# RIVM-bioinformatics/TrueConsense

Measured on NVIDIA B200. Metric: aligned_bases_per_sec_pileup_consensus, higher is better.
Workload: dtype int32

## Files before the change

### trueconsense_b200/csrc/cuda/call.cu

```cuda
#include <stdlib.h>

#include "tc_common.cuh"

__device__ __forceinline__ double pct(int c, int cov) { return __dmul_rn(__ddiv_rn((double)c, (double)cov), 100.0); }
__device__ __forceinline__ bool within(double a, double b, double maxdist) { return fabs(__dsub_rn(a, b)) <= maxdist; }

struct ranked5 { int cnt[5]; char let[5]; };

__device__ __forceinline__ void rank5(const int c[5], ranked5& r) {
    const int asc[5] = {'A', 'T', 'C', 'G', 'X'};
#pragma unroll
    for (int i = 0; i < 5; ++i) {
        int beat = 0;
#pragma unroll
        for (int j = 0; j < 5; ++j)
            if (j != i && (c[j] > c[i] || (c[j] == c[i] && asc[j] > asc[i]))) ++beat;
#pragma unroll
        for (int k = 0; k < 5; ++k)
            if (beat == k) { r.cnt[k] = c[i]; r.let[k] = (char)asc[i]; }
    }
}

__device__ __forceinline__ char iupac_of_mask(int m) {
    switch (m) {
// ... 126 lines not shown
    nn = min(nn, end);
    xrun[j] = nn - k;
    if (nn == end) flags[j] |= TC_CF_XRUN_OFF_END;
}

__global__ void is_ambiguous_kernel(const uint8_t* __restrict__ letters, const int32_t* __restrict__ cnts,
                                    const int32_t* __restrict__ cov, int64_t n, double maxdist, uint8_t* __restrict__ out) {
    int64_t i = (int64_t)blockIdx.x * blockDim.x + threadIdx.x;
    if (i >= n) return;
    char let[4]; int cnt[4];
#pragma unroll
    for (int k = 0; k < 4; ++k) { let[k] = (char)letters[k * n + i]; cnt[k] = cnts[k * n + i]; }
    out[i] = (uint8_t)is_ambiguous(let, cnt, cov[i], maxdist);
}

__global__ void list_candidates_kernel(const uint8_t* __restrict__ flags, int L, int32_t* __restrict__ out, int cap, int32_t* __restrict__ n_out) {
    const int j = blockIdx.x * blockDim.x + threadIdx.x;
    if (j < L && (flags[j] & TC_CF_INS_CANDIDATE)) {
        const int slot = atomicAdd(n_out, 1);
        if (slot < cap) out[slot] = j + 1;
    }
}

__global__ void rank_sort_kernel(const int32_t* __restrict__ in, const int32_t* __restrict__ n_in, int cap, int32_t* __restrict__ out) {
    const int n = min(*n_in, cap);
    for (int i = blockIdx.x * blockDim.x + threadIdx.x; i < n; i += gridDim.x * blockDim.x) {
        const int v = in[i];
        int rank = 0;
        for (int k = 0; k < n; ++k) rank += in[k] < v;
        out[rank] = v;
    }
}

static int call_table(tc_ctx_t* ctx, const int32_t* counts, int32_t ref_len, const int32_t* d_contig_start, int32_t n_contigs,
                      const tc_call_params_t* p, const tc_call_table_t* t, cudaStream_t s) {
    const size_t L = (size_t)ref_len;
    int rc;
    call_args a;
    a.counts = (const int32_t*)tc_stage_in(ctx, SLOT_COUNTS, counts, sizeof(int32_t) * TC_NROWS * L, s, &rc);
    if (rc) return rc;
    a.L = ref_len; a.mincov = p->mincov; a.include_ambig = p->include_ambig;
    a.maxdist = p->ambig_maxdist; a.mdel_pct = p->minority_del_pct; a.ins_pct = p->insert_pct;
    struct out_t { void* user; void* dev; size_t bytes; int slot; };
    out_t outs[6] = {
        {t->call_char, nullptr, L, SLOT_CALL_A}, {t->flags, nullptr, L, SLOT_CALL_B}, {t->xrun, nullptr, 4 * L, SLOT_CALL_C},
        {t->rank_letter, nullptr, 4 * L, SLOT_CALL_D}, {t->rank_count, nullptr, 16 * L, SLOT_CALL_E}, {t->ambig_char, nullptr, L, SLOT_CALL_F}};
// ... 79 lines not shown
    const int32_t* dc = (const int32_t*)tc_stage_in(ctx, SLOT_TMP_B, cnts, 16 * (size_t)n, s, &rc); if (rc) return rc;
    const int32_t* dv = (const int32_t*)tc_stage_in(ctx, SLOT_TMP_C, cov, 4 * (size_t)n, s, &rc); if (rc) return rc;
    bool out_dev = tc_is_device_ptr(out_char);
    uint8_t* d_out = out_dev ? out_char : (uint8_t*)tc_dev_buf(ctx, SLOT_CALL_F, (size_t)n);
    if (!d_out) return TC_ERR_NOMEM;
    is_ambiguous_kernel<<<(unsigned)((n + 255) / 256), 256, 0, s>>>(dl, dc, dv, n, maxdist, d_out);
    TC_LAUNCH_CHECK();
    if (!out_dev) {
        TC_D2H(out_char, d_out, (size_t)n, s);
        TC_CUDA(cudaStreamSynchronize(s));
    }
    return TC_OK;
}

int tc_candidates_enqueue(tc_ctx* ctx, const uint8_t* d_flags, int32_t ref_len, int32_t cap, int32_t** d_count, int32_t** d_sorted, cudaStream_t s) {
    int32_t* d_buf = (int32_t*)tc_dev_buf(ctx, SLOT_TMP_B, 4 * (2 * (size_t)cap + 1) + 64);
    if (!d_buf) return TC_ERR_NOMEM;
    int32_t* d_cnt = d_buf + cap;
    TC_CUDA(cudaMemsetAsync(d_cnt, 0, 4, s));
    list_candidates_kernel<<<(unsigned)((ref_len + 255) / 256), 256, 0, s>>>(d_flags, ref_len, d_buf, cap, d_cnt);
    TC_LAUNCH_CHECK();
    rank_sort_kernel<<<32, 256, 0, s>>>(d_buf, d_cnt, cap, d_cnt + 1);
    TC_LAUNCH_CHECK();
    *d_count = d_cnt; *d_sorted = d_cnt + 1;
    return TC_OK;
}

TC_API int tc_list_insert_candidates(tc_ctx_t* ctx, const uint8_t* flags, int32_t ref_len, int32_t* cand_pos, int32_t cap,
                                     int32_t* n_out, void* stream) {
    if (!ctx) return TC_ERR_ARG;
    if (!flags || !cand_pos || !n_out || ref_len <= 0 || cap < 0) return tc_fail(ctx, TC_ERR_ARG, "bad argument");
    cudaStream_t s = (cudaStream_t)stream;
    TC_CUDA(cudaSetDevice(ctx->device));
    int rc;
    const uint8_t* df = (const uint8_t*)tc_stage_in(ctx, SLOT_TMP_A, flags, (size_t)ref_len, s, &rc); if (rc) return rc;
    int32_t *d_cnt, *d_sorted;
    rc = tc_candidates_enqueue(ctx, df, ref_len, cap, &d_cnt, &d_sorted, s);
// ... 21 lines not shown
```

### trueconsense_b200/csrc/cuda/inserts.cu

```cuda
#include <cub/device/device_segmented_radix_sort.cuh>

#include <memory>
#include <new>

#include "tc_common.cuh"

constexpr int INS_TILE = 256;
constexpr uint64_t KEY_NONE = ~0ull;
constexpr int INS_TBL = 4096;
constexpr int INS_BASES_FIXED = 64;

struct ins_args {
    dreads r;
    const int32_t* cand;
    int n_cand;
    const int32_t* n_cand_dev;
    uint32_t flag_filter; int min_mapq, min_bq, ignore_orphans; long long max_depth;
    int32_t span_hint;
    int32_t* range;
    uint32_t* range_off;
    const int64_t* seg_off;
    const int32_t* tile_cand;
    const int32_t* tile_first;
    int32_t* tile_sel;
    int32_t* tile_last;
    uint64_t* ent_key; int32_t* ent_indel; int32_t* ent_qpos; uint8_t* ent_head;
    uint8_t* ent_sel;
    uint8_t* ent_q;
    uint8_t* pair_q; unsigned long long pair_cap; unsigned long long* pair_bump;
    int olap_mode;
    int32_t* seg_count;
    int32_t* pair_any;
    int32_t* overflow;
    const int32_t* layout;
    uint8_t* bases_fixed;
    tc_status* status;
};

__device__ __forceinline__ int ins_ncand(const ins_args& a) { return a.n_cand_dev ? min(*a.n_cand_dev, a.n_cand) : a.n_cand; }

__global__ void max_span_kernel(dreads r, tc_status* status) {
    int64_t i = (int64_t)blockIdx.x * blockDim.x + threadIdx.x;
    int span = 0;
    if (i < r.n) {
        if (i > 0 && r.pos[i] < r.pos[i - 1]) atomicCAS(&status->err, 0, TC_ERR_UNSORTED);
        for (uint32_t k = r.cigar_off[i]; k < r.cigar_off[i + 1]; ++k) {
            uint32_t c = r.cigar[k];
            if (op_consumes_ref(c & 15u)) span += (int)(c >> 4);
        }
    }
    span = __reduce_max_sync(0xffffffffu, span);
    if ((threadIdx.x & 31) == 0 && span > 0) atomicMax(&status->max_span, span);
}

__device__ __forceinline__ int warp_lower_bound(const int32_t* __restrict__ pos, int64_t n, int v, int lane) {
    int64_t lo = 0, hi = n;
    while (hi > lo) {
        const int64_t step = (hi - lo + 31) / 32;
        const int64_t i = lo + (int64_t)lane * step;
        const bool ge = i >= hi || pos[i] >= v;
        const unsigned m = __ballot_sync(0xffffffffu, ge);
        if (m == 0u) { lo = lo + 31 * step + 1; continue; }
        const int first = __ffs(m) - 1;
        if (first == 0) return (int)lo;
        hi = min(hi, lo + (int64_t)first * step);
        lo = lo + (int64_t)(first - 1) * step + 1;
    }
    return (int)lo;
}

__global__ void cand_range_kernel(ins_args a) {
    const int ci = blockIdx.x * (blockDim.x >> 5) + (threadIdx.x >> 5);
    const int lane = threadIdx.x & 31;
    if (ci >= ins_ncand(a)) return;
    const int c = a.cand[ci] - 1;
    const int ms = max(a.span_hint > 0 ? a.span_hint : a.status->max_span, 1);
    const int lo = warp_lower_bound(a.r.pos, a.r.n, c - ms + 1, lane);
    const int hi = max(lo, warp_lower_bound(a.r.pos, a.r.n, c + 1, lane));
    if (lane == 0) {
        a.range[2 * ci] = lo;
        a.range[2 * ci + 1] = hi;
        a.range_off[4 * ci] = a.r.seq_off[lo]; a.range_off[4 * ci + 1] = a.r.seq_off[hi];
        a.range_off[4 * ci + 2] = a.r.cigar_off[lo]; a.range_off[4 * ci + 3] = a.r.cigar_off[hi];
    }
}

__device__ __forceinline__ uint64_t mix_key(uint64_t h, uint64_t v) {
    h ^= v + 0x9e3779b97f4a7c15ull + (h << 6) + (h >> 2);
    h *= 0xff51afd7ed558ccdull;
    h ^= h >> 33;
    return h;
}

__device__ __forceinline__ char base_char_upper(uint32_t code, bool rev) {
// ... 168 lines not shown
#pragma unroll
    for (int o = 1; o < 32; o <<= 1) { const int t = __shfl_up_sync(0xffffffffu, m, o); if (lane >= o) m = max(m, t); }
    int prev = __shfl_up_sync(0xffffffffu, m, 1);
    if (lane == 0) prev = -1;
    if (lane == 31) wlast[warp] = m;
    if (lane == 0) wsum[warp] = __popc(bal);
    __syncthreads();
    long long rank = base_s + __popc(bal & ((1u << lane) - 1));
    prev = max(prev, prev_s);
    for (int w = 0; w < warp; ++w) { rank += wsum[w]; prev = max(prev, wlast[w]); }
    bool admitted = false;
    if (sel) {
        const bool first_at_start = prev < 0 || a.r.pos[prev] != a.r.pos[r];
        admitted = first_at_start || rank < a.max_depth;
    }
    if (a.min_bq > 0) {
        if (r < hi && admitted) a.ent_sel[slot] = (uint8_t)(es | 4);
        return;
    }
    if (emit && !admitted) a.ent_key[slot] = KEY_NONE;
    const int n_adm = __syncthreads_count(emit && admitted);
    if (threadIdx.x == 0 && n_adm) atomicAdd(&a.seg_count[ci], n_adm);
}

__device__ __forceinline__ uint32_t wang_hash(uint32_t key) {
    key += ~(key << 15); key ^= (key >> 10); key += (key << 3); key ^= (key >> 6); key += ~(key << 11); key ^= (key >> 16);
    return key;
}

struct cwalk { const uint32_t* cig; const uint32_t* end; long long icig, iseq, iref; };

__device__ int iref2iseq_set(cwalk& w, long long pos) {
    if (pos < 0) return -1;
    w.icig = 0; w.iseq = 0; w.iref = 0;
    while (w.cig < w.end) {
        const uint32_t cig = *w.cig & 15u; const long long ncig = (long long)(*w.cig >> 4);
// ... 99 lines not shown
        for (uint32_t k = a.r.cigar_off[r]; k < a.r.cigar_off[r + 1]; ++k) { const uint32_t c = a.r.cigar[k]; if (op_consumes_ref(c & 15u)) end += (int)(c >> 4); }
        if (mp >= end) return false;
    }
    return true;
}

__global__ void __launch_bounds__(1024) ins_pair_kernel(ins_args a) {
    extern __shared__ __align__(16) unsigned char pair_smem[];
    unsigned int* tmin = reinterpret_cast<unsigned int*>(pair_smem);
    unsigned int* tmax = tmin + PAIR_TBL;
    unsigned short* tcnt = reinterpret_cast<unsigned short*>(tmax + PAIR_TBL);
    __shared__ int over_s, nadm_s;
    const int ci = blockIdx.x;
    if (ci >= ins_ncand(a)) return;
    if (a.layout && a.layout[2]) return;
    const int64_t off = a.seg_off[ci];
    const int lo = a.range[2 * ci];
    const int n = a.range[2 * ci + 1] - lo;
    const bool pairing = a.olap_mode != 1 && a.r.qname_hash && a.r.mpos && a.r.isize && a.pair_any[ci];
    if (threadIdx.x == 0) { over_s = 0; nadm_s = 0; }
    if (pairing) {
        for (int i = threadIdx.x; i < PAIR_TBL; i += blockDim.x) { tmin[i] = 0u; tmax[i] = 0u; tcnt[i] = 0; }
        __syncthreads();
        auto is_event = [&](int i, bool& push) -> bool {
            const uint8_t es = a.ent_sel[off + i];
            if (!(es & 1)) return false;
            if (!(es & 4)) { push = false; return true; }
            push = true;
            return true;
        };
        for (int pass = 0; pass < 2; ++pass) {
            for (int i = threadIdx.x; i < n; i += blockDim.x) {
                bool push;
                if (!is_event(i, push) || push != (pass == 0)) continue;
                const uint32_t r = (uint32_t)(lo + i);
                if (push && !(a.r.flag[r] & 2u)) continue;
                const unsigned long long k = a.r.qname_hash[r];
                unsigned h = (unsigned)(k ^ (k >> 31)) & (PAIR_TBL - 1);
                int probes = 0;
                for (;;) {
                    const unsigned cur = push ? atomicCAS(&tmin[h], 0u, (unsigned)i + 1u) : tmin[h];
                    if (cur == 0u && !push) break;
                    if (cur == 0u || a.r.qname_hash[lo + cur - 1] == k) {
                        atomicMin(&tmin[h], (unsigned)i + 1u); atomicMax(&tmax[h], (unsigned)i + 1u);
                        atomicAdd(reinterpret_cast<unsigned int*>(tcnt) + (h >> 1), (h & 1) ? 0x10000u : 1u);
                        break;
                    }
                    h = (h + 1) & (PAIR_TBL - 1);
                    if (++probes >= PAIR_TBL * 3 / 4) { over_s = 1; break; }
                }
            }
            __syncthreads();
        }
        __syncthreads();
        if (over_s) { if (threadIdx.x == 0) atomicCAS(&a.status->err, 0, TC_ERR_CAPACITY); return; }
        for (int h = threadIdx.x; h < PAIR_TBL; h += blockDim.x) {
            const int cnt = tcnt[h];
            if (cnt < 2) continue;
            const int first = (int)tmin[h] - 1, last = (int)tmax[h] - 1;
            const unsigned long long k = a.r.qname_hash[lo + first];
            int stored = -1;
            int seen = 0;
            for (int i = first; i <= last && seen < cnt; i = (cnt == 2 && i == first) ? last : i + 1) {
                bool push;
                if (!is_event(i, push)) continue;
                const uint32_t r = (uint32_t)(lo + i);
                if (a.r.qname_hash[r] != k || (push && !(a.r.flag[r] & 2u))) continue;
                ++seen;
                if (!push) { stored = -1; continue; }
                if (!olap_eligible(a, r)) continue;
                bool has_span = false;
                for (uint32_t q = a.r.cigar_off[r]; q < a.r.cigar_off[r + 1] && !has_span; ++q) { const uint32_t c = a.r.cigar[q]; has_span = op_consumes_ref(c & 15u) && (c >> 4) > 0; }
                if (!has_span) continue;
                if (stored < 0) {
                    const int mp = a.r.mpos[r];
                    if (mp >= a.r.pos[r] || ((a.r.flag[r] & 1u) && mp == -1)) stored = i;
                    continue;
                }
                const int64_t sa = off + stored, sb = off + i;
                const uint32_t ra = (uint32_t)(lo + stored);
                const int la = a.r.l_seq[ra], lb = a.r.l_seq[r];
                const unsigned long long at = atomicAdd(a.pair_bump, (unsigned long long)(la + lb));
                if (at + (unsigned long long)(la + lb) <= a.pair_cap) {
                    uint8_t* aq = a.pair_q + at; uint8_t* bq = aq + la;
                    const uint8_t* ga = a.r.qual + 8ull * a.r.seq_off[ra]; const uint8_t* gb = a.r.qual + 8ull * a.r.seq_off[r];
                    for (int q = 0; q < la; ++q) aq[q] = ga[q];
                    for (int q = 0; q < lb; ++q) bq[q] = gb[q];
                    tweak_pair(a, ra, r, aq, bq, a.olap_mode);
                    if ((a.ent_sel[sa] & 2) && a.ent_qpos[sa] < la) a.ent_q[sa] = aq[a.ent_qpos[sa]];
                    if ((a.ent_sel[sb] & 2) && a.ent_qpos[sb] < lb) a.ent_q[sb] = bq[a.ent_qpos[sb]];
                } else atomicOr(a.overflow, 2);
                stored = -1;
            }
        }
        __syncthreads();
    }
    int mine = 0;
    for (int i = threadIdx.x; i < n; i += blockDim.x) {
        const uint8_t es = a.ent_sel[off + i];
        const bool ok = (es & 6) == 6 && (int)a.ent_q[off + i] >= a.min_bq;
        if (!ok) a.ent_key[off + i] = KEY_NONE;
        mine += ok ? 1 : 0;
    }
    mine = __reduce_add_sync(0xffffffffu, mine);
    if ((threadIdx.x & 31) == 0 && mine) atomicAdd(&nadm_s, mine);
    __syncthreads();
    if (threadIdx.x == 0) a.seg_count[ci] = nadm_s;
}

__device__ __forceinline__ bool same_entry(const ins_args& a, int lo, int64_t off, uint32_t e1, uint32_t e2) {
    if (a.ent_head[e1] != a.ent_head[e2] || a.ent_indel[e1] != a.ent_indel[e2]) return false;
// ... 21 lines not shown
        const uint32_t e = (uint32_t)off + (uint32_t)(0xffffffffull - (best & 0xffffffffull));
        out.mode_count = (int32_t)(best >> 32);
        out.first_read = (int32_t)(a.range[2 * ci] + (int64_t)e - off);
        out.head = a.ent_head[e];
        out.indel = a.ent_indel[e];
        out.bases_off = (int64_t)e;
        if (out.indel > 0 && out.indel <= INS_BASES_FIXED) {
            const read_syms rs = read_syms_of(a, (uint32_t)out.first_read);
            const int q = a.ent_qpos[e];
            for (int j = 1; j <= out.indel; ++j) a.bases_fixed[(size_t)ci * INS_BASES_FIXED + j - 1] = sym_char(rs.sym(q + j));
        }
    }
    calls[ci] = out;
}

__global__ void __launch_bounds__(1024) ins_count_kernel(ins_args a, tc_insert_call_t* __restrict__ calls) {
    extern __shared__ __align__(16) unsigned char ins_smem[];
    unsigned long long* tkey = reinterpret_cast<unsigned long long*>(ins_smem);
    unsigned int* tcnt = reinterpret_cast<unsigned int*>(tkey + INS_TBL);
    unsigned int* tfirst = tcnt + INS_TBL;
    __shared__ unsigned long long best_s;
    __shared__ int over_s, hashed_s;
    const int ci = blockIdx.x;
    if (ci >= ins_ncand(a)) return;
    if (a.layout && a.layout[2]) return;
    const int64_t off = a.seg_off[ci];
    const int lo = a.range[2 * ci];
    const int n = a.range[2 * ci + 1] - lo;
    for (int i = threadIdx.x; i < INS_TBL; i += blockDim.x) { tkey[i] = KEY_NONE; tcnt[i] = 0; tfirst[i] = 0xffffffffu; }
    if (threadIdx.x == 0) { best_s = 0ull; over_s = 0; hashed_s = 0; }
    __syncthreads();
    for (int base = 0; base < n; base += 4 * (int)blockDim.x) {
        unsigned long long kk[4];
#pragma unroll
        for (int u = 0; u < 4; ++u) {
            const int i = base + u * (int)blockDim.x + (int)threadIdx.x;
            kk[u] = i < n ? a.ent_key[off + i] : KEY_NONE;
        }
#pragma unroll
        for (int u = 0; u < 4; ++u) {
            const int i = base + u * (int)blockDim.x + (int)threadIdx.x;
            const unsigned long long k = kk[u];
            const unsigned grp = __match_any_sync(0xffffffffu, k);
            if (k == KEY_NONE || (__ffs(grp) - 1) != (int)(threadIdx.x & 31)) continue;
            if (!(k >> 62)) hashed_s = 1;
            unsigned h = (unsigned)(k ^ (k >> 29)) & (INS_TBL - 1);
            int probes = 0;
            for (;;) {
                const unsigned long long old = atomicCAS(&tkey[h], KEY_NONE, k);
                if (old == KEY_NONE || old == k) { atomicAdd(&tcnt[h], (unsigned)__popc(grp)); atomicMin(&tfirst[h], (unsigned)i); break; }
                h = (h + 1) & (INS_TBL - 1);
                if (++probes >= INS_TBL * 7 / 8) { over_s = 1; break; }
            }
        }
    }
    __syncthreads();
    if (over_s) { if (threadIdx.x == 0) atomicOr(a.overflow, 1); return; }
    if (hashed_s)
    for (int i = threadIdx.x; i < n; i += blockDim.x) {
        const unsigned long long k = a.ent_key[off + i];
        if (k == KEY_NONE || (k >> 62)) continue;
        unsigned h = (unsigned)(k ^ (k >> 29)) & (INS_TBL - 1);
        while (tkey[h] != k) h = (h + 1) & (INS_TBL - 1);
        const unsigned f = tfirst[h];
        if (f != (unsigned)i && !same_entry(a, lo, off, (uint32_t)(off + f), (uint32_t)(off + i))) atomicCAS(&a.status->err, 0, TC_ERR_RANGE);
    }
    unsigned long long best = 0ull;
    for (int i = threadIdx.x; i < INS_TBL; i += blockDim.x)
        if (tcnt[i]) best = max(best, ((unsigned long long)tcnt[i] << 32) | (0xffffffffull - (unsigned long long)tfirst[i]));
    atomicMax(&best_s, best);
    __syncthreads();
    if (threadIdx.x == 0) write_call(a, ci, a.seg_count[ci], best_s, calls);
}

__global__ void __launch_bounds__(1024) ins_mode_kernel(ins_args a, const uint64_t* __restrict__ skey, const uint32_t* __restrict__ sidx,
                                                        tc_insert_call_t* __restrict__ calls) {
    __shared__ unsigned long long best_s;
    const int ci = blockIdx.x;
    const int64_t off = a.seg_off[ci];
    const int lo_read = a.range[2 * ci];
// ... 39 lines not shown
}

static ins_block ins_block_of(int n_cand, bool with_extra) {
    static_assert(sizeof(tc_status) <= 64, "tc_status outgrew its place in the results block");
    ins_block b;
    b.layout = 64; b.over = 80; b.bump = 88;
    b.extra = with_extra ? 128 : 0;
    b.seg = with_extra ? b.extra + 4 * (TC_RB_EXTRA_CAND + (size_t)n_cand) : 96;
    b.calls = b.seg + ((4 * (2 * (size_t)n_cand + 2) + 15) & ~(size_t)15);
    b.fixed = b.calls + sizeof(tc_insert_call_t) * (size_t)n_cand;
    b.bytes = b.fixed + (size_t)n_cand * INS_BASES_FIXED;
    return b;
}

static int ins_bind(tc_ctx* ctx, ins_args& a, uint8_t* d_rb, const ins_block& rb, size_t T, size_t NT, int n_cand, const tc_pileup_params_t* p) {
    const size_t bytes = T * (8 + 4 + 4 + 1 + 1 + 1) + NT * 12 + ((size_t)n_cand + 1) * 16 + 256 + 16;
    uint8_t* slab = (uint8_t*)tc_dev_buf(ctx, SLOT_INS_D, bytes);
    if (!slab) return TC_ERR_NOMEM;
    a.ent_key = (uint64_t*)slab;
    int64_t* d_off = (int64_t*)(a.ent_key + T);
    a.seg_off = d_off;
    a.ent_indel = (int32_t*)(d_off + n_cand + 1); a.ent_qpos = a.ent_indel + T;
    int32_t* d_tcand = a.ent_qpos + T; int32_t* d_tfirst = d_tcand + NT;
    a.tile_cand = d_tcand; a.tile_first = d_tfirst;
    a.tile_sel = d_tfirst + n_cand + 1; a.tile_last = a.tile_sel + NT;
    a.ent_head = (uint8_t*)(a.tile_last + NT); a.ent_sel = a.ent_head + T; a.ent_q = a.ent_sel + T;
    a.seg_count = (int32_t*)(d_rb + rb.seg); a.pair_any = a.seg_count + n_cand + 1; a.overflow = (int32_t*)(d_rb + rb.over);
    a.bases_fixed = d_rb + rb.fixed;
    if (ctx->pair_cap <= 0) ctx->pair_cap = 1 << 22;
    a.pair_bump = (unsigned long long*)(d_rb + rb.bump); a.pair_cap = (unsigned long long)ctx->pair_cap;
    a.pair_q = (uint8_t*)tc_dev_buf(ctx, SLOT_INS_F, (size_t)ctx->pair_cap);
    if (!a.pair_q) return TC_ERR_NOMEM;
    a.flag_filter = p->flag_filter; a.min_mapq = p->min_mapq; a.min_bq = p->min_base_quality; a.ignore_orphans = p->ignore_orphans;
    a.olap_mode = (p->reserved >> 8) & 3;
    a.max_depth = p->max_depth > 0 ? p->max_depth : (1ll << 62);
    return TC_OK;
}

static int ins_layout_dev(tc_ctx* ctx, ins_args& a, uint8_t* d_rb, const ins_block& rb, size_t T, size_t NT, const tc_status* pileup_status,
                          cudaStream_t s) {
    int32_t* d_layout = (int32_t*)(d_rb + rb.layout);
// ... 9 lines not shown
        ins_select_kernel<<<tiles, INS_TILE, 0, s>>>(a);
        TC_LAUNCH_CHECK();
        ins_admit_kernel<<<tiles, INS_TILE, 0, s>>>(a);
        TC_LAUNCH_CHECK();
    }
    if (a.min_bq > 0) {
        const size_t smem = (size_t)PAIR_TBL * 10;
        if (!(ctx->ins_attr_set & 2)) {
            TC_CUDA(cudaFuncSetAttribute(ins_pair_kernel, cudaFuncAttributeMaxDynamicSharedMemorySize, (int)smem));
            ctx->ins_attr_set |= 2;
        }
        ins_pair_kernel<<<grid, 1024, smem, s>>>(a);
        TC_LAUNCH_CHECK();
    }
    if (d_calls) {
        const size_t smem = (size_t)INS_TBL * 16;
        if (!(ctx->ins_attr_set & 1)) {
            TC_CUDA(cudaFuncSetAttribute(ins_count_kernel, cudaFuncAttributeMaxDynamicSharedMemorySize, (int)smem));
            ctx->ins_attr_set |= 1;
        }
        ins_count_kernel<<<grid, 1024, smem, s>>>(a, d_calls);
        TC_LAUNCH_CHECK();
    }
    return TC_OK;
}

static int ins_check_status(tc_ctx* ctx, const tc_status& st) {
    if (st.err == TC_ERR_UNSORTED) return tc_fail(ctx, TC_ERR_UNSORTED, "Unsorted input. Pileup aborts");
    if (st.err) return tc_fail(ctx, st.err, "insertion key collision or device-side failure %d", st.err);
    return TC_OK;
}

static int ins_place_bases(tc_ctx* ctx, tc_insert_call_t* calls, int n, const uint8_t* fixed, uint8_t* bases, int64_t bases_cap,
                           int64_t* need_out = nullptr) {
    int64_t need = 0;
    for (int i = 0; i < n; ++i) {
// ... 72 lines not shown
        const ins_block rb = ins_block_of(n_cand, false);
        uint8_t* d_rb = (uint8_t*)tc_dev_buf(ctx, SLOT_INS_E, rb.bytes + 16);
        int32_t* d_cand = (int32_t*)tc_dev_buf(ctx, SLOT_INS_A, 4 * (size_t)n_cand);
        int32_t* d_range = (int32_t*)tc_dev_buf(ctx, SLOT_INS_B, 24 * (size_t)n_cand);
        if (!d_rb || !d_cand || !d_range) return TC_ERR_NOMEM;
        a.status = (tc_status*)d_rb;
        TC_CUDA(cudaMemsetAsync(d_rb, 0, rb.calls, s));
        TC_CUDA(cudaMemcpyAsync(d_cand, cand_pos, 4 * (size_t)n_cand, cudaMemcpyHostToDevice, s));
        ctx->h2d_bytes += 4 * (int64_t)n_cand;
        a.span_hint = bounded ? reads->max_ref_span : 0;
        if (a.span_hint == 0) {
            max_span_kernel<<<(unsigned)((n + 255) / 256), 256, 0, s>>>(a.r, a.status);
            TC_LAUNCH_CHECK();
        }
        a.cand = d_cand; a.n_cand = n_cand; a.range = d_range; a.range_off = (uint32_t*)(d_range + 2 * (size_t)n_cand);
        cand_range_kernel<<<(n_cand + 3) / 4, 128, 0, s>>>(a);
        TC_LAUNCH_CHECK();
        const bool spec = !(host_seq || host_qual || host_cig || host_mate) && q.kernel != 2 && !(q.reserved & 1);
        if (ctx->ins_slot_cap <= 0) ctx->ins_slot_cap = 1 << 16;
        std::unique_ptr<int64_t[]> h_off;
        std::unique_ptr<int32_t[]> h_tfirst, h_tcand;
        int64_t total = ctx->ins_slot_cap;
        int n_tiles = (int)(total / INS_TILE) + n_cand + 1;
        if (!spec) {
            auto h_range = host_array<int32_t>(6 * (size_t)n_cand);
            h_off = host_array<int64_t>((size_t)n_cand + 1);
            h_tfirst = host_array<int32_t>((size_t)n_cand + 1);
            if (!h_range || !h_off || !h_tfirst) return tc_fail(ctx, TC_ERR_NOMEM, "out of host memory");
            if ((rc = ins_copy(ctx, h_range.get(), d_range, 24 * (size_t)n_cand, cudaMemcpyDeviceToHost, s, "range readback")) ||
                (rc = ins_sync(ctx, s, "range readback")))
                return rc;
// ... 137 lines not shown
    if (rc) return rc;
    const int64_t n = a.r.n;
    const ins_block rb = ins_block_of(cap, true);
    if (rb.bytes > TC_HOST_SCRATCH) return tc_fail(ctx, TC_ERR_ARG, "candidate capacity %d too large for the pinned results block", cap);
    uint8_t* d_rb = (uint8_t*)tc_dev_buf(ctx, SLOT_INS_E, rb.bytes + 16);
    int32_t* d_range = (int32_t*)tc_dev_buf(ctx, SLOT_INS_B, 24 * (size_t)cap);
    if (!d_rb || !d_range) return TC_ERR_NOMEM;
    TC_CUDA(cudaMemsetAsync(d_rb, 0, rb.calls, s));
    a.span_hint = reads->max_ref_span > 0 ? reads->max_ref_span : 0;
    a.status = (tc_status*)d_rb;
    if (a.span_hint == 0 && n > 0) {
        max_span_kernel<<<(unsigned)((n + 255) / 256), 256, 0, s>>>(a.r, a.status);
        TC_LAUNCH_CHECK();
    }
    a.cand = d_cand; a.n_cand = cap; a.n_cand_dev = d_ncand; a.range = d_range; a.range_off = (uint32_t*)(d_range + 2 * (size_t)cap);
    cand_range_kernel<<<(cap + 3) / 4, 128, 0, s>>>(a);
    TC_LAUNCH_CHECK();
    if (ctx->ins_slot_cap <= 0) ctx->ins_slot_cap = 1 << 16;
    const size_t T = (size_t)ctx->ins_slot_cap, NT = T / INS_TILE + (size_t)cap + 1;
    if ((rc = ins_bind(ctx, a, d_rb, rb, T, NT, cap, p)) || (rc = ins_layout_dev(ctx, a, d_rb, rb, T, NT, d_pileup_status, s))) return rc;
    if (n > 0 && (rc = ins_enqueue_count(ctx, a, (unsigned)NT, cap, (tc_insert_call_t*)(d_rb + rb.calls), s))) return rc;
    TC_CUDA(cudaMemcpyAsync(host_block, d_rb, rb.bytes, cudaMemcpyDeviceToHost, s));
    ctx->d2h_bytes += (int64_t)rb.bytes;
    pend->rb = rb; pend->cap = cap; pend->n_reads = n;
    return TC_OK;
}

int tc_inserts_finish_dev(tc_ctx* ctx, const tc_ins_pending* pend, const void* host_block, tc_status* pileup_status, int32_t* cands, int32_t* n_cand,
                          tc_insert_call_t* calls, uint8_t* bases, int64_t bases_cap, int* fit) {
    const uint8_t* pin = (const uint8_t*)host_block;
    const ins_block& rb = pend->rb;
// ... 22 lines not shown
```

Baseline: 1228 billion.

## Replace candidate sort with decoupled-lookback scan and add per-tile insert pre-aggregation

Candidate listing now uses a single-pass ordered compaction with a decoupled lookback prefix scan instead of atomic append followed by a quadratic rank sort. The insert counting path is split into a per-tile shared-memory hash pre-aggregation kernel and a merge kernel that works on deduplicated keys, which shrinks global hashing work. cand_range now computes its two binary searches in parallel warps. The pair kernel returns early when pairing is not needed, and the quality filter moves into the admission step. Together these add more scratch memory and extra kernels, and the scan relies on spin-waiting between blocks.

Measured after the change: 1282 billion, median of 6. 4.4% higher.

```diff
diff --git a/trueconsense_b200/csrc/cuda/call.cu b/trueconsense_b200/csrc/cuda/call.cu
--- a/trueconsense_b200/csrc/cuda/call.cu
+++ b/trueconsense_b200/csrc/cuda/call.cu
@@ -164,22 +164,60 @@
     out[i] = (uint8_t)is_ambiguous(let, cnt, cov[i], maxdist);
 }
 
-__global__ void list_candidates_kernel(const uint8_t* __restrict__ flags, int L, int32_t* __restrict__ out, int cap, int32_t* __restrict__ n_out) {
-    const int j = blockIdx.x * blockDim.x + threadIdx.x;
-    if (j < L && (flags[j] & TC_CF_INS_CANDIDATE)) {
-        const int slot = atomicAdd(n_out, 1);
-        if (slot < cap) out[slot] = j + 1;
-    }
-}
-
-__global__ void rank_sort_kernel(const int32_t* __restrict__ in, const int32_t* __restrict__ n_in, int cap, int32_t* __restrict__ out) {
-    const int n = min(*n_in, cap);
-    for (int i = blockIdx.x * blockDim.x + threadIdx.x; i < n; i += gridDim.x * blockDim.x) {
-        const int v = in[i];
-        int rank = 0;
-        for (int k = 0; k < n; ++k) rank += in[k] < v;
-        out[rank] = v;
-    }
+constexpr int LC_THREADS = 256;
+constexpr int LC_COLS = 4 * LC_THREADS;
+
+__global__ void __launch_bounds__(LC_THREADS) list_candidates_kernel(const uint8_t* __restrict__ flags, int L, int32_t* __restrict__ out, int cap,
+                                                                     int32_t* __restrict__ n_out, unsigned long long* __restrict__ state) {
+    __shared__ int wsum[LC_THREADS / 32];
+    __shared__ int vb_s, excl_s;
+    const int lane = threadIdx.x & 31, warp = threadIdx.x >> 5;
+    if (threadIdx.x == 0) vb_s = (int)atomicAdd(reinterpret_cast<unsigned int*>(state), 1u);
+    __syncthreads();
+    const int vb = vb_s;
+    const int j = vb * LC_COLS + 4 * (int)threadIdx.x;
+    unsigned m = 0;
+#pragma unroll
+    for (int u = 0; u < 4; ++u)
+        if (j + u < L && (flags[j + u] & TC_CF_INS_CANDIDATE)) m |= 1u << u;
+    const int c = __popc(m);
+    int x = c;
+#pragma unroll
+    for (int o = 1; o < 32; o <<= 1) { const int t = __shfl_up_sync(0xffffffffu, x, o); if (lane >= o) x += t; }
+    if (lane == 31) wsum[warp] = x;
+    __syncthreads();
+    if (warp == 0) {
+        int w = lane < LC_THREADS / 32 ? wsum[lane] : 0;
+#pragma unroll
+        for (int o = 1; o < 32; o <<= 1) { const int t = __shfl_up_sync(0xffffffffu, w, o); if (lane >= o) w += t; }
+        if (lane < LC_THREADS / 32) wsum[lane] = w;
+        const int total = __shfl_sync(0xffffffffu, w, LC_THREADS / 32 - 1);
+        volatile unsigned long long* st = state + 1;
+        int excl = 0;
+        if (vb > 0) {
+            if (lane == 0) st[vb] = (1ull << 32) | (unsigned)total;
+            for (int top = vb - 1;;) {
+                const int q = top - lane;
+                const unsigned long long v = q >= 0 ? st[q] : (2ull << 32);
+                const unsigned inc = __ballot_sync(0xffffffffu, (v >> 32) == 2);
+                const unsigned need = inc ? ((inc & (0u - inc)) << 1) - 1u : ~0u;
+                if (__ballot_sync(0xffffffffu, (v >> 32) == 0) & need) continue;
+                excl += (int)__reduce_add_sync(0xffffffffu, ((need >> lane) & 1u) ? (unsigned)v : 0u);
+                if (inc) break;
+                top -= 32;
+            }
+        }
+        if (lane == 0) {
+            st[vb] = (2ull << 32) | (unsigned)(excl + total);
+            excl_s = excl;
+            if (vb == (int)gridDim.x - 1) *n_out = excl + total;
+        }
+    }
+    __syncthreads();
+    int at = excl_s + x - c + (warp ? wsum[warp - 1] : 0);
+#pragma unroll
+    for (int u = 0; u < 4; ++u)
+        if ((m >> u) & 1u) { if (at < cap) out[at] = j + u + 1; ++at; }
 }
 
 static int call_table(tc_ctx_t* ctx, const int32_t* counts, int32_t ref_len, const int32_t* d_contig_start, int32_t n_contigs,
@@ -289,13 +327,14 @@
 }
 
 int tc_candidates_enqueue(tc_ctx* ctx, const uint8_t* d_flags, int32_t ref_len, int32_t cap, int32_t** d_count, int32_t** d_sorted, cudaStream_t s) {
-    int32_t* d_buf = (int32_t*)tc_dev_buf(ctx, SLOT_TMP_B, 4 * (2 * (size_t)cap + 1) + 64);
+    const unsigned blocks = (unsigned)((ref_len + LC_COLS - 1) / LC_COLS);
+    const size_t state_at = (4 * ((size_t)cap + 1) + 15) & ~(size_t)15, state_bytes = 8 * ((size_t)blocks + 1);
+    uint8_t* d_buf = (uint8_t*)tc_dev_buf(ctx, SLOT_TMP_B, state_at + state_bytes + 64);
     if (!d_buf) return TC_ERR_NOMEM;
-    int32_t* d_cnt = d_buf + cap;
-    TC_CUDA(cudaMemsetAsync(d_cnt, 0, 4, s));
-    list_candidates_kernel<<<(unsigned)((ref_len + 255) / 256), 256, 0, s>>>(d_flags, ref_len, d_buf, cap, d_cnt);
-    TC_LAUNCH_CHECK();
-    rank_sort_kernel<<<32, 256, 0, s>>>(d_buf, d_cnt, cap, d_cnt + 1);
+    unsigned long long* d_state = (unsigned long long*)(d_buf + state_at);
+    TC_CUDA(cudaMemsetAsync(d_state, 0, state_bytes, s));
+    int32_t* d_cnt = (int32_t*)d_buf;
+    list_candidates_kernel<<<blocks, LC_THREADS, 0, s>>>(d_flags, ref_len, d_cnt + 1, cap, d_cnt, d_state);
     TC_LAUNCH_CHECK();
     *d_count = d_cnt; *d_sorted = d_cnt + 1;
     return TC_OK;
diff --git a/trueconsense_b200/csrc/cuda/inserts.cu b/trueconsense_b200/csrc/cuda/inserts.cu
--- a/trueconsense_b200/csrc/cuda/inserts.cu
+++ b/trueconsense_b200/csrc/cuda/inserts.cu
@@ -24,6 +24,9 @@
     const int32_t* tile_first;
     int32_t* tile_sel;
     int32_t* tile_last;
+    uint64_t* lst_key;
+    uint64_t* lst_cf;
+    int32_t* tile_nd;
     uint64_t* ent_key; int32_t* ent_indel; int32_t* ent_qpos; uint8_t* ent_head;
     uint8_t* ent_sel;
     uint8_t* ent_q;
@@ -39,6 +42,10 @@
 
 __device__ __forceinline__ int ins_ncand(const ins_args& a) { return a.n_cand_dev ? min(*a.n_cand_dev, a.n_cand) : a.n_cand; }
 
+__device__ __forceinline__ bool ins_pairing(const ins_args& a, int ci) {
+    return a.min_bq > 0 && a.olap_mode != 1 && a.r.qname_hash && a.r.mpos && a.r.isize && a.pair_any[ci];
+}
+
 __global__ void max_span_kernel(dreads r, tc_status* status) {
     int64_t i = (int64_t)blockIdx.x * blockDim.x + threadIdx.x;
     int span = 0;
@@ -69,15 +76,24 @@
     return (int)lo;
 }
 
-__global__ void cand_range_kernel(ins_args a) {
-    const int ci = blockIdx.x * (blockDim.x >> 5) + (threadIdx.x >> 5);
+constexpr int RANGE_CANDS = 4;
+
+__global__ void __launch_bounds__(64 * RANGE_CANDS) cand_range_kernel(ins_args a) {
+    __shared__ int bound_s[RANGE_CANDS][2];
+    const int slot = threadIdx.x >> 6, which = (threadIdx.x >> 5) & 1;
+    const int ci = blockIdx.x * RANGE_CANDS + slot;
     const int lane = threadIdx.x & 31;
-    if (ci >= ins_ncand(a)) return;
-    const int c = a.cand[ci] - 1;
-    const int ms = max(a.span_hint > 0 ? a.span_hint : a.status->max_span, 1);
-    const int lo = warp_lower_bound(a.r.pos, a.r.n, c - ms + 1, lane);
-    const int hi = max(lo, warp_lower_bound(a.r.pos, a.r.n, c + 1, lane));
-    if (lane == 0) {
+    const bool live = ci < ins_ncand(a);
+    if (live) {
+        const int c = a.cand[ci] - 1;
+        const int ms = max(a.span_hint > 0 ? a.span_hint : a.status->max_span, 1);
+        const int b = warp_lower_bound(a.r.pos, a.r.n, which ? c + 1 : c - ms + 1, lane);
+        if (lane == 0) bound_s[slot][which] = b;
+    }
+    __syncthreads();
+    if (live && which == 0 && lane == 0) {
+        const int lo = bound_s[slot][0];
+        const int hi = max(lo, bound_s[slot][1]);
         a.range[2 * ci] = lo;
         a.range[2 * ci + 1] = hi;
         a.range_off[4 * ci] = a.r.seq_off[lo]; a.range_off[4 * ci + 1] = a.r.seq_off[hi];
@@ -276,12 +292,13 @@
         const bool first_at_start = prev < 0 || a.r.pos[prev] != a.r.pos[r];
         admitted = first_at_start || rank < a.max_depth;
     }
-    if (a.min_bq > 0) {
+    if (ins_pairing(a, ci)) {
         if (r < hi && admitted) a.ent_sel[slot] = (uint8_t)(es | 4);
         return;
     }
-    if (emit && !admitted) a.ent_key[slot] = KEY_NONE;
-    const int n_adm = __syncthreads_count(emit && admitted);
+    const bool ok = emit && admitted && (a.min_bq == 0 || (int)a.ent_q[slot] >= a.min_bq);
+    if (emit && !ok) a.ent_key[slot] = KEY_NONE;
+    const int n_adm = __syncthreads_count(ok);
     if (threadIdx.x == 0 && n_adm) atomicAdd(&a.seg_count[ci], n_adm);
 }
 
@@ -411,87 +428,85 @@
     const int ci = blockIdx.x;
     if (ci >= ins_ncand(a)) return;
     if (a.layout && a.layout[2]) return;
+    if (!ins_pairing(a, ci)) return;
     const int64_t off = a.seg_off[ci];
     const int lo = a.range[2 * ci];
     const int n = a.range[2 * ci + 1] - lo;
-    const bool pairing = a.olap_mode != 1 && a.r.qname_hash && a.r.mpos && a.r.isize && a.pair_any[ci];
     if (threadIdx.x == 0) { over_s = 0; nadm_s = 0; }
-    if (pairing) {
-        for (int i = threadIdx.x; i < PAIR_TBL; i += blockDim.x) { tmin[i] = 0u; tmax[i] = 0u; tcnt[i] = 0; }
+    for (int i = threadIdx.x; i < PAIR_TBL; i += blockDim.x) { tmin[i] = 0u; tmax[i] = 0u; tcnt[i] = 0; }
+    __syncthreads();
+    auto is_event = [&](int i, bool& push) -> bool {
+        const uint8_t es = a.ent_sel[off + i];
+        if (!(es & 1)) return false;
+        if (!(es & 4)) { push = false; return true; }
+        push = true;
+        return true;
+    };
+    for (int pass = 0; pass < 2; ++pass) {
+        for (int i = threadIdx.x; i < n; i += blockDim.x) {
+            bool push;
+            if (!is_event(i, push) || push != (pass == 0)) continue;
+            const uint32_t r = (uint32_t)(lo + i);
+            if (push && !(a.r.flag[r] & 2u)) continue;
+            const unsigned long long k = a.r.qname_hash[r];
+            unsigned h = (unsigned)(k ^ (k >> 31)) & (PAIR_TBL - 1);
+            int probes = 0;
+            for (;;) {
+                const unsigned cur = push ? atomicCAS(&tmin[h], 0u, (unsigned)i + 1u) : tmin[h];
+                if (cur == 0u && !push) break;
+                if (cur == 0u || a.r.qname_hash[lo + cur - 1] == k) {
+                    atomicMin(&tmin[h], (unsigned)i + 1u); atomicMax(&tmax[h], (unsigned)i + 1u);
+                    atomicAdd(reinterpret_cast<unsigned int*>(tcnt) + (h >> 1), (h & 1) ? 0x10000u : 1u);
+                    break;
+                }
+                h = (h + 1) & (PAIR_TBL - 1);
+                if (++probes >= PAIR_TBL * 3 / 4) { over_s = 1; break; }
+            }
+        }
         __syncthreads();
-        auto is_event = [&](int i, bool& push) -> bool {
-            const uint8_t es = a.ent_sel[off + i];
-            if (!(es & 1)) return false;
-            if (!(es & 4)) { push = false; return true; }
-            push = true;
-            return true;
-        };
-        for (int pass = 0; pass < 2; ++pass) {
-            for (int i = threadIdx.x; i < n; i += blockDim.x) {
-                bool push;
-                if (!is_event(i, push) || push != (pass == 0)) continue;
-                const uint32_t r = (uint32_t)(lo + i);
-                if (push && !(a.r.flag[r] & 2u)) continue;
-                const unsigned long long k = a.r.qname_hash[r];
-                unsigned h = (unsigned)(k ^ (k >> 31)) & (PAIR_TBL - 1);
-                int probes = 0;
-                for (;;) {
-                    const unsigned cur = push ? atomicCAS(&tmin[h], 0u, (unsigned)i + 1u) : tmin[h];
-                    if (cur == 0u && !push) break;
-                    if (cur == 0u || a.r.qname_hash[lo + cur - 1] == k) {
-                        atomicMin(&tmin[h], (unsigned)i + 1u); atomicMax(&tmax[h], (unsigned)i + 1u);
-                        atomicAdd(reinterpret_cast<unsigned int*>(tcnt) + (h >> 1), (h & 1) ? 0x10000u : 1u);
-                        break;
-                    }
-                    h = (h + 1) & (PAIR_TBL - 1);
-                    if (++probes >= PAIR_TBL * 3 / 4) { over_s = 1; break; }
-                }
+    }
+    __syncthreads();
+    if (over_s) { if (threadIdx.x == 0) atomicCAS(&a.status->err, 0, TC_ERR_CAPACITY); return; }
+    for (int h = threadIdx.x; h < PAIR_TBL; h += blockDim.x) {
+        const int cnt = tcnt[h];
+        if (cnt < 2) continue;
+        const int first = (int)tmin[h] - 1, last = (int)tmax[h] - 1;
+        const unsigned long long k = a.r.qname_hash[lo + first];
+        int stored = -1;
+        int seen = 0;
+        for (int i = first; i <= last && seen < cnt; i = (cnt == 2 && i == first) ? last : i + 1) {
+            bool push;
+            if (!is_event(i, push)) continue;
+            const uint32_t r = (uint32_t)(lo + i);
+            if (a.r.qname_hash[r] != k || (push && !(a.r.flag[r] & 2u))) continue;
+            ++seen;
+            if (!push) { stored = -1; continue; }
+            if (!olap_eligible(a, r)) continue;
+            bool has_span = false;
+            for (uint32_t q = a.r.cigar_off[r]; q < a.r.cigar_off[r + 1] && !has_span; ++q) { const uint32_t c = a.r.cigar[q]; has_span = op_consumes_ref(c & 15u) && (c >> 4) > 0; }
+            if (!has_span) continue;
+            if (stored < 0) {
+                const int mp = a.r.mpos[r];
+                if (mp >= a.r.pos[r] || ((a.r.flag[r] & 1u) && mp == -1)) stored = i;
+                continue;
             }
-            __syncthreads();
-        }
-        __syncthreads();
-        if (over_s) { if (threadIdx.x == 0) atomicCAS(&a.status->err, 0, TC_ERR_CAPACITY); return; }
-        for (int h = threadIdx.x; h < PAIR_TBL; h += blockDim.x) {
-            const int cnt = tcnt[h];
-            if (cnt < 2) continue;
-            const int first = (int)tmin[h] - 1, last = (int)tmax[h] - 1;
-            const unsigned long long k = a.r.qname_hash[lo + first];
-            int stored = -1;
-            int seen = 0;
-            for (int i = first; i <= last && seen < cnt; i = (cnt == 2 && i == first) ? last : i + 1) {
-                bool push;
-                if (!is_event(i, push)) continue;
-                const uint32_t r = (uint32_t)(lo + i);
-                if (a.r.qname_hash[r] != k || (push && !(a.r.flag[r] & 2u))) continue;
-                ++seen;
-                if (!push) { stored = -1; continue; }
-                if (!olap_eligible(a, r)) continue;
-                bool has_span = false;
-                for (uint32_t q = a.r.cigar_off[r]; q < a.r.cigar_off[r + 1] && !has_span; ++q) { const uint32_t c = a.r.cigar[q]; has_span = op_consumes_ref(c & 15u) && (c >> 4) > 0; }
-                if (!has_span) continue;
-                if (stored < 0) {
-                    const int mp = a.r.mpos[r];
-                    if (mp >= a.r.pos[r] || ((a.r.flag[r] & 1u) && mp == -1)) stored = i;
-                    continue;
-                }
-                const int64_t sa = off + stored, sb = off + i;
-                const uint32_t ra = (uint32_t)(lo + stored);
-                const int la = a.r.l_seq[ra], lb = a.r.l_seq[r];
-                const unsigned long long at = atomicAdd(a.pair_bump, (unsigned long long)(la + lb));
-                if (at + (unsigned long long)(la + lb) <= a.pair_cap) {
-                    uint8_t* aq = a.pair_q + at; uint8_t* bq = aq + la;
-                    const uint8_t* ga = a.r.qual + 8ull * a.r.seq_off[ra]; const uint8_t* gb = a.r.qual + 8ull * a.r.seq_off[r];
-                    for (int q = 0; q < la; ++q) aq[q] = ga[q];
-                    for (int q = 0; q < lb; ++q) bq[q] = gb[q];
-                    tweak_pair(a, ra, r, aq, bq, a.olap_mode);
-                    if ((a.ent_sel[sa] & 2) && a.ent_qpos[sa] < la) a.ent_q[sa] = aq[a.ent_qpos[sa]];
-                    if ((a.ent_sel[sb] & 2) && a.ent_qpos[sb] < lb) a.ent_q[sb] = bq[a.ent_qpos[sb]];
-                } else atomicOr(a.overflow, 2);
-                stored = -1;
-            }
-        }
-        __syncthreads();
-    }
+            const int64_t sa = off + stored, sb = off + i;
+            const uint32_t ra = (uint32_t)(lo + stored);
+            const int la = a.r.l_seq[ra], lb = a.r.l_seq[r];
+            const unsigned long long at = atomicAdd(a.pair_bump, (unsigned long long)(la + lb));
+            if (at + (unsigned long long)(la + lb) <= a.pair_cap) {
+                uint8_t* aq = a.pair_q + at; uint8_t* bq = aq + la;
+                const uint8_t* ga = a.r.qual + 8ull * a.r.seq_off[ra]; const uint8_t* gb = a.r.qual + 8ull * a.r.seq_off[r];
+                for (int q = 0; q < la; ++q) aq[q] = ga[q];
+                for (int q = 0; q < lb; ++q) bq[q] = gb[q];
+                tweak_pair(a, ra, r, aq, bq, a.olap_mode);
+                if ((a.ent_sel[sa] & 2) && a.ent_qpos[sa] < la) a.ent_q[sa] = aq[a.ent_qpos[sa]];
+                if ((a.ent_sel[sb] & 2) && a.ent_qpos[sb] < lb) a.ent_q[sb] = bq[a.ent_qpos[sb]];
+            } else atomicOr(a.overflow, 2);
+            stored = -1;
+        }
+    }
+    __syncthreads();
     int mine = 0;
     for (int i = threadIdx.x; i < n; i += blockDim.x) {
         const uint8_t es = a.ent_sel[off + i];
@@ -543,7 +558,50 @@
     calls[ci] = out;
 }
 
-__global__ void __launch_bounds__(1024) ins_count_kernel(ins_args a, tc_insert_call_t* __restrict__ calls) {
+constexpr int TILE_TBL = 2 * INS_TILE;
+
+__global__ void __launch_bounds__(INS_TILE) ins_tile_count_kernel(ins_args a) {
+    __shared__ unsigned long long tkey[TILE_TBL];
+    __shared__ unsigned int tcnt[TILE_TBL], tfirst[TILE_TBL];
+    __shared__ int nd_s, hashed_s;
+    const int tile = blockIdx.x;
+    if (a.layout && tile >= a.layout[0]) return;
+    const int ci = a.tile_cand[tile];
+    const int lo = a.range[2 * ci], hi = a.range[2 * ci + 1];
+    const int64_t off = a.seg_off[ci];
+    const int i = (tile - a.tile_first[ci]) * INS_TILE + (int)threadIdx.x;
+    for (int h = threadIdx.x; h < TILE_TBL; h += INS_TILE) { tkey[h] = KEY_NONE; tcnt[h] = 0; tfirst[h] = 0xffffffffu; }
+    if (threadIdx.x == 0) { nd_s = 0; hashed_s = 0; }
+    __syncthreads();
+    const unsigned long long k = lo + i < hi ? a.ent_key[off + i] : KEY_NONE;
+    const unsigned grp = __match_any_sync(0xffffffffu, k);
+    const unsigned h0 = (unsigned)(k ^ (k >> 29)) & (TILE_TBL - 1);
+    if (k != KEY_NONE && (__ffs(grp) - 1) == (int)(threadIdx.x & 31)) {
+        if (!(k >> 62)) hashed_s = 1;
+        for (unsigned h = h0;; h = (h + 1) & (TILE_TBL - 1)) {
+            const unsigned long long old = atomicCAS(&tkey[h], KEY_NONE, k);
+            if (old == KEY_NONE || old == k) { atomicAdd(&tcnt[h], (unsigned)__popc(grp)); atomicMin(&tfirst[h], (unsigned)i); break; }
+        }
+    }
+    __syncthreads();
+    if (hashed_s && k != KEY_NONE && !(k >> 62)) {
+        unsigned h = h0;
+        while (tkey[h] != k) h = (h + 1) & (TILE_TBL - 1);
+        const unsigned f = tfirst[h];
+        if (f != (unsigned)i && !same_entry(a, lo, off, (uint32_t)(off + f), (uint32_t)(off + i))) atomicCAS(&a.status->err, 0, TC_ERR_RANGE);
+    }
+    const int64_t base = off + i - (int)threadIdx.x;
+    for (int h = threadIdx.x; h < TILE_TBL; h += INS_TILE) {
+        if (!tcnt[h]) continue;
+        const int j = atomicAdd(&nd_s, 1);
+        a.lst_key[base + j] = tkey[h];
+        a.lst_cf[base + j] = ((unsigned long long)tcnt[h] << 32) | tfirst[h];
+    }
+    __syncthreads();
+    if (threadIdx.x == 0) a.tile_nd[tile] = nd_s;
+}
+
+__global__ void __launch_bounds__(1024) ins_merge_kernel(ins_args a, tc_insert_call_t* __restrict__ calls) {
     extern __shared__ __align__(16) unsigned char ins_smem[];
     unsigned long long* tkey = reinterpret_cast<unsigned long long*>(ins_smem);
     unsigned int* tcnt = reinterpret_cast<unsigned int*>(tkey + INS_TBL);
@@ -555,29 +613,22 @@
     if (a.layout && a.layout[2]) return;
     const int64_t off = a.seg_off[ci];
     const int lo = a.range[2 * ci];
-    const int n = a.range[2 * ci + 1] - lo;
+    const int t0 = a.tile_first[ci], t1 = a.tile_first[ci + 1];
     for (int i = threadIdx.x; i < INS_TBL; i += blockDim.x) { tkey[i] = KEY_NONE; tcnt[i] = 0; tfirst[i] = 0xffffffffu; }
     if (threadIdx.x == 0) { best_s = 0ull; over_s = 0; hashed_s = 0; }
     __syncthreads();
-    for (int base = 0; base < n; base += 4 * (int)blockDim.x) {
-        unsigned long long kk[4];
-#pragma unroll
-        for (int u = 0; u < 4; ++u) {
-            const int i = base + u * (int)blockDim.x + (int)threadIdx.x;
-            kk[u] = i < n ? a.ent_key[off + i] : KEY_NONE;
-        }
-#pragma unroll
-        for (int u = 0; u < 4; ++u) {
-            const int i = base + u * (int)blockDim.x + (int)threadIdx.x;
-            const unsigned long long k = kk[u];
-            const unsigned grp = __match_any_sync(0xffffffffu, k);
-            if (k == KEY_NONE || (__ffs(grp) - 1) != (int)(threadIdx.x & 31)) continue;
+    const int lane = threadIdx.x & 31, warps = (int)blockDim.x >> 5;
+    for (int t = t0 + ((int)threadIdx.x >> 5); t < t1; t += warps) {
+        const int nd = a.tile_nd[t];
+        const int64_t base = off + (int64_t)(t - t0) * INS_TILE;
+        for (int j = lane; j < nd; j += 32) {
+            const unsigned long long k = a.lst_key[base + j], cf = a.lst_cf[base + j];
             if (!(k >> 62)) hashed_s = 1;
             unsigned h = (unsigned)(k ^ (k >> 29)) & (INS_TBL - 1);
             int probes = 0;
             for (;;) {
                 const unsigned long long old = atomicCAS(&tkey[h], KEY_NONE, k);
-                if (old == KEY_NONE || old == k) { atomicAdd(&tcnt[h], (unsigned)__popc(grp)); atomicMin(&tfirst[h], (unsigned)i); break; }
+                if (old == KEY_NONE || old == k) { atomicAdd(&tcnt[h], (unsigned)(cf >> 32)); atomicMin(&tfirst[h], (unsigned)cf); break; }
                 h = (h + 1) & (INS_TBL - 1);
                 if (++probes >= INS_TBL * 7 / 8) { over_s = 1; break; }
             }
@@ -586,13 +637,18 @@
     __syncthreads();
     if (over_s) { if (threadIdx.x == 0) atomicOr(a.overflow, 1); return; }
     if (hashed_s)
-    for (int i = threadIdx.x; i < n; i += blockDim.x) {
-        const unsigned long long k = a.ent_key[off + i];
-        if (k == KEY_NONE || (k >> 62)) continue;
-        unsigned h = (unsigned)(k ^ (k >> 29)) & (INS_TBL - 1);
-        while (tkey[h] != k) h = (h + 1) & (INS_TBL - 1);
-        const unsigned f = tfirst[h];
-        if (f != (unsigned)i && !same_entry(a, lo, off, (uint32_t)(off + f), (uint32_t)(off + i))) atomicCAS(&a.status->err, 0, TC_ERR_RANGE);
+    for (int t = t0 + ((int)threadIdx.x >> 5); t < t1; t += warps) {
+        const int nd = a.tile_nd[t];
+        const int64_t base = off + (int64_t)(t - t0) * INS_TILE;
+        for (int j = lane; j < nd; j += 32) {
+            const unsigned long long k = a.lst_key[base + j];
+            if (k >> 62) continue;
+            const unsigned g = (unsigned)a.lst_cf[base + j];
+            unsigned h = (unsigned)(k ^ (k >> 29)) & (INS_TBL - 1);
+            while (tkey[h] != k) h = (h + 1) & (INS_TBL - 1);
+            const unsigned f = tfirst[h];
+            if (f != g && !same_entry(a, lo, off, (uint32_t)(off + f), (uint32_t)(off + g))) atomicCAS(&a.status->err, 0, TC_ERR_RANGE);
+        }
     }
     unsigned long long best = 0ull;
     for (int i = threadIdx.x; i < INS_TBL; i += blockDim.x)
@@ -662,17 +718,17 @@
 }
 
 static int ins_bind(tc_ctx* ctx, ins_args& a, uint8_t* d_rb, const ins_block& rb, size_t T, size_t NT, int n_cand, const tc_pileup_params_t* p) {
-    const size_t bytes = T * (8 + 4 + 4 + 1 + 1 + 1) + NT * 12 + ((size_t)n_cand + 1) * 16 + 256 + 16;
+    const size_t bytes = T * (8 + 8 + 8 + 4 + 4 + 1 + 1 + 1) + NT * 16 + ((size_t)n_cand + 1) * 16 + 256 + 16;
     uint8_t* slab = (uint8_t*)tc_dev_buf(ctx, SLOT_INS_D, bytes);
     if (!slab) return TC_ERR_NOMEM;
-    a.ent_key = (uint64_t*)slab;
-    int64_t* d_off = (int64_t*)(a.ent_key + T);
+    a.ent_key = (uint64_t*)slab; a.lst_key = a.ent_key + T; a.lst_cf = a.lst_key + T;
+    int64_t* d_off = (int64_t*)(a.lst_cf + T);
     a.seg_off = d_off;
     a.ent_indel = (int32_t*)(d_off + n_cand + 1); a.ent_qpos = a.ent_indel + T;
     int32_t* d_tcand = a.ent_qpos + T; int32_t* d_tfirst = d_tcand + NT;
     a.tile_cand = d_tcand; a.tile_first = d_tfirst;
-    a.tile_sel = d_tfirst + n_cand + 1; a.tile_last = a.tile_sel + NT;
-    a.ent_head = (uint8_t*)(a.tile_last + NT); a.ent_sel = a.ent_head + T; a.ent_q = a.ent_sel + T;
+    a.tile_sel = d_tfirst + n_cand + 1; a.tile_last = a.tile_sel + NT; a.tile_nd = a.tile_last + NT;
+    a.ent_head = (uint8_t*)(a.tile_nd + NT); a.ent_sel = a.ent_head + T; a.ent_q = a.ent_sel + T;
     a.seg_count = (int32_t*)(d_rb + rb.seg); a.pair_any = a.seg_count + n_cand + 1; a.overflow = (int32_t*)(d_rb + rb.over);
     a.bases_fixed = d_rb + rb.fixed;
     if (ctx->pair_cap <= 0) ctx->pair_cap = 1 << 22;
@@ -712,12 +768,16 @@
         TC_LAUNCH_CHECK();
     }
     if (d_calls) {
+        if (tiles) {
+            ins_tile_count_kernel<<<tiles, INS_TILE, 0, s>>>(a);
+            TC_LAUNCH_CHECK();
+        }
         const size_t smem = (size_t)INS_TBL * 16;
         if (!(ctx->ins_attr_set & 1)) {
-            TC_CUDA(cudaFuncSetAttribute(ins_count_kernel, cudaFuncAttributeMaxDynamicSharedMemorySize, (int)smem));
+            TC_CUDA(cudaFuncSetAttribute(ins_merge_kernel, cudaFuncAttributeMaxDynamicSharedMemorySize, (int)smem));
             ctx->ins_attr_set |= 1;
         }
-        ins_count_kernel<<<grid, 1024, smem, s>>>(a, d_calls);
+        ins_merge_kernel<<<grid, 1024, smem, s>>>(a, d_calls);
         TC_LAUNCH_CHECK();
     }
     return TC_OK;
@@ -820,7 +880,7 @@
             TC_LAUNCH_CHECK();
         }
         a.cand = d_cand; a.n_cand = n_cand; a.range = d_range; a.range_off = (uint32_t*)(d_range + 2 * (size_t)n_cand);
-        cand_range_kernel<<<(n_cand + 3) / 4, 128, 0, s>>>(a);
+        cand_range_kernel<<<(n_cand + RANGE_CANDS - 1) / RANGE_CANDS, 64 * RANGE_CANDS, 0, s>>>(a);
         TC_LAUNCH_CHECK();
         const bool spec = !(host_seq || host_qual || host_cig || host_mate) && q.kernel != 2 && !(q.reserved & 1);
         if (ctx->ins_slot_cap <= 0) ctx->ins_slot_cap = 1 << 16;
@@ -988,7 +1048,7 @@
         TC_LAUNCH_CHECK();
     }
     a.cand = d_cand; a.n_cand = cap; a.n_cand_dev = d_ncand; a.range = d_range; a.range_off = (uint32_t*)(d_range + 2 * (size_t)cap);
-    cand_range_kernel<<<(cap + 3) / 4, 128, 0, s>>>(a);
+    cand_range_kernel<<<(cap + RANGE_CANDS - 1) / RANGE_CANDS, 64 * RANGE_CANDS, 0, s>>>(a);
     TC_LAUNCH_CHECK();
     if (ctx->ins_slot_cap <= 0) ctx->ins_slot_cap = 1 << 16;
     const size_t T = (size_t)ctx->ins_slot_cap, NT = T / INS_TILE + (size_t)cap + 1;
```
